# chjj/lcdb

Measured on AMD Instinct MI355X. Metric: device-resident GiB/s Snappy encode+decode, 4 KiB blocks, 1/2/4/8 MI355X, higher is better.
Workload: dtype u8

## Files before the change

lcdb_amd/csrc/lgs_api.cpp:

```cpp

#include <hip/hip_runtime.h>

#include <stdarg.h>
#include <stdint.h>
#include <stdio.h>
#include <stdlib.h>
#include <string.h>
#include <unistd.h>

#include <algorithm>
#include <atomic>
#include <chrono>
#include <condition_variable>
#include <deque>
#include <functional>
#include <memory>
#include <mutex>
#include <thread>
#include <unordered_map>
#include <vector>

#include "lgs_host.h"

namespace lgs {
// ... 1075 lines not shown
                        const uint32_t* d_key_len, const uint32_t* d_first, uint32_t nfilters,
                        int bits_per_key, uint8_t* d_out, const uint64_t* d_out_off,
                        void* stream) {
  if (nfilters == 0) return LGS_OK;
  if (!d_keys || !d_key_off || !d_key_len || !d_first || !d_out || !d_out_off)
    return fail(LGS_EINVAL, "NULL argument");
  if (bits_per_key < 0 || bits_per_key > kMaxBitsPerKey)
    return fail(LGS_EINVAL, "bits_per_key %d out of range", bits_per_key);
  LGS_HIP(launch_bloom_build(d_keys, d_key_off, d_key_len, d_first, nfilters,
                             (uint32_t)bits_per_key, bloom_k(bits_per_key), d_out, d_out_off,
                             0, (hipStream_t)stream));
  return LGS_OK;
}

int lgs_bloom_match_dev(const uint8_t* d_filters, const uint64_t* d_filter_off,
                        const uint32_t* d_filter_len, const uint32_t* d_query_filter,
                        const uint8_t* d_keys, const uint64_t* d_key_off,
                        const uint32_t* d_key_len, uint8_t* d_match, uint32_t nq, void* stream) {
  if (nq == 0) return LGS_OK;
  if (!d_filters || !d_filter_off || !d_filter_len || !d_query_filter || !d_keys || !d_key_off ||
      !d_key_len || !d_match)
    return fail(LGS_EINVAL, "NULL argument");
  LGS_HIP(launch_bloom_match(d_filters, d_filter_off, d_filter_len, d_query_filter, d_keys,
                             d_key_off, d_key_len, d_match, nq, (hipStream_t)stream));
  return LGS_OK;
}

int lgs_bloom_build_host(const uint8_t* keys, const uint64_t* key_off, const uint32_t* key_len,
                         const uint32_t* first, uint32_t nfilters, int bits_per_key,
                         uint8_t* out, const uint64_t* out_off) {
  if (nfilters == 0) return LGS_OK;
  if (!keys || !key_off || !key_len || !first || !out || !out_off)
    return fail(LGS_EINVAL, "NULL argument");
  if (bits_per_key < 0 || bits_per_key > kMaxBitsPerKey)
    return fail(LGS_EINVAL, "bits_per_key %d out of range", bits_per_key);
  for (uint32_t f = 0; f < nfilters; ++f)
    if (first[f + 1] < first[f]) return fail(LGS_EINVAL, "first[] decreases at filter %u", f);
  Lease lease(batch_pool());
  LGS_TRY(lease.acquire());
  Ctx& c = lease.ctx();
  const uint32_t nkeys = first[nfilters] - first[0];
  const uint32_t k0 = first[0];
  size_t key_bytes = 0, filt_bytes = 0;
  for (uint32_t i = k0; i < k0 + nkeys; ++i) key_bytes += key_len[i];
  for (uint32_t f = 0; f < nfilters; ++f)
    filt_bytes += lgs_bloom_filter_size(first[f + 1] - first[f], bits_per_key);
  Layout L;
  const size_t o_keys = L.take(key_bytes + 16);
  const size_t o_koff = L.take(8 * (size_t)nkeys);
  const size_t o_klen = L.take(4 * (size_t)nkeys);
  const size_t o_first = L.take(4 * ((size_t)nfilters + 1));
  const size_t o_foff = L.take(8 * (size_t)nfilters);
  const size_t up_end = L.at;
  const size_t o_filt = L.take(filt_bytes + 16);
  const size_t down_end = L.at;
  LGS_TRY(ctx_reserve(c, down_end, down_end));
  uint8_t* h = c.h_buf;
  uint8_t* d = c.d_buf;
  uint64_t* koff = (uint64_t*)(h + o_koff);
  uint32_t* klen = (uint32_t*)(h + o_klen);
  uint32_t* fst = (uint32_t*)(h + o_first);
  uint64_t* foff = (uint64_t*)(h + o_foff);
  size_t at = o_keys;
  for (uint32_t j = 0; j < nkeys; ++j) {
    memcpy(h + at, keys + key_off[k0 + j], key_len[k0 + j]);
    koff[j] = at;
    klen[j] = key_len[k0 + j];
    at += key_len[k0 + j];
  }
  memset(h + at, 0, 16);
  size_t fat = 0;
  for (uint32_t f = 0; f <= nfilters; ++f) fst[f] = first[f] - k0;
  for (uint32_t f = 0; f < nfilters; ++f) {
    foff[f] = fat;
    fat += lgs_bloom_filter_size(first[f + 1] - first[f], bits_per_key);
  }
  LGS_HIP(hipMemcpyAsync(d, h, up_end, hipMemcpyHostToDevice, c.stream));
  LGS_HIP(launch_bloom_build(d, (const uint64_t*)(d + o_koff), (const uint32_t*)(d + o_klen),
                             (const uint32_t*)(d + o_first), nfilters, (uint32_t)bits_per_key,
                             bloom_k(bits_per_key), d + o_filt, (const uint64_t*)(d + o_foff),
                             0, c.stream));
  LGS_HIP(hipMemcpyAsync(h + o_filt, d + o_filt, filt_bytes, hipMemcpyDeviceToHost, c.stream));
  LGS_HIP(hipStreamSynchronize(c.stream));
  for (uint32_t f = 0; f < nfilters; ++f)
    memcpy(out + out_off[f], h + o_filt + foff[f],
           lgs_bloom_filter_size(first[f + 1] - first[f], bits_per_key));
  return LGS_OK;
}

int lgs_bloom_match_host(const uint8_t* filters, const uint64_t* filter_off,
                         const uint32_t* filter_len, uint32_t nfilters,
                         const uint32_t* query_filter, const uint8_t* keys,
                         const uint64_t* key_off, const uint32_t* key_len, uint32_t nq,
                         uint8_t* match) {
  if (nq == 0) return LGS_OK;
  if (!filters || !filter_off || !filter_len || !query_filter || !keys || !key_off || !key_len ||
      !match)
    return fail(LGS_EINVAL, "NULL argument");
  for (uint32_t q = 0; q < nq; ++q)
    if (query_filter[q] >= nfilters)
      return fail(LGS_EINVAL, "query %u names filter %u of %u", q, query_filter[q], nfilters);
  Lease lease(batch_pool());
  LGS_TRY(lease.acquire());
  Ctx& c = lease.ctx();
  size_t fb = 0, kb = 0;
  for (uint32_t f = 0; f < nfilters; ++f) fb += filter_len[f];
  for (uint32_t q = 0; q < nq; ++q) kb += key_len[q];
  Layout L;
  const size_t o_f = L.take(fb + 16);
  const size_t o_foff = L.take(8 * (size_t)nfilters);
  const size_t o_flen = L.take(4 * (size_t)nfilters);
  const size_t o_qf = L.take(4 * (size_t)nq);
  const size_t o_k = L.take(kb + 16);
  const size_t o_koff = L.take(8 * (size_t)nq);
  const size_t o_klen = L.take(4 * (size_t)nq);
  const size_t up_end = L.at;
  const size_t o_m = L.take(nq);
  const size_t down_end = L.at;
  LGS_TRY(ctx_reserve(c, down_end, down_end));
  uint8_t* h = c.h_buf;
  uint8_t* d = c.d_buf;
  uint64_t* foff = (uint64_t*)(h + o_foff);
  uint32_t* flen = (uint32_t*)(h + o_flen);
  size_t at = 0;
  for (uint32_t f = 0; f < nfilters; ++f) {
    memcpy(h + o_f + at, filters + filter_off[f], filter_len[f]);
    foff[f] = at;
    flen[f] = filter_len[f];
    at += filter_len[f];
  }
  memset(h + o_f + at, 0, 16);
  memcpy(h + o_qf, query_filter, 4 * (size_t)nq);
  stage_keys(keys, key_off, key_len, nq, h + o_k, (uint64_t*)(h + o_koff), (uint32_t*)(h + o_klen));
  LGS_HIP(hipMemcpyAsync(d, h, up_end, hipMemcpyHostToDevice, c.stream));
  LGS_HIP(launch_bloom_match(d + o_f, (const uint64_t*)(d + o_foff), (const uint32_t*)(d + o_flen),
                             (const uint32_t*)(d + o_qf), d + o_k, (const uint64_t*)(d + o_koff),
                             (const uint32_t*)(d + o_klen), d + o_m, nq, c.stream));
  LGS_HIP(hipMemcpyAsync(h + o_m, d + o_m, nq, hipMemcpyDeviceToHost, c.stream));
  LGS_HIP(hipStreamSynchronize(c.stream));
  memcpy(match, h + o_m, nq);
  return LGS_OK;
}

int lgs_device_count(void) { return visible_devices(); }

int lgs_set_device(int device) {
  int count = lgs_device_count();
  if (device < 0 || device >= count)
    return fail(LGS_ENODEV, "device %d not present (%d visible)", device, count);
  t_want_device = device;
  return LGS_OK;
}

const char* lgs_last_error(void) { return t_err; }

const char* lgs_version(void) { return "lcdb_gpu_snappy 0.1 gfx950"; }

}
```

lcdb_amd/csrc/lgs_encode.hip:

```cpp
#include "lgs_device.h"
#include "lgs_probe_hooks.h"
#include "lgs_launch.h"
#include "lgs_service.h"

namespace lgs {

__constant__ ProbeTable kProbe = ProbeTable();

struct OutSlot {
  __amdgpu_buffer_rsrc_t r;
  __device__ void put(uint32_t soff, uint32_t voff, uint32_t v) const {
    __builtin_amdgcn_raw_buffer_store_b8((uint8_t)v, r, (int)voff, (int)soff, 0);
  }
  __device__ void put2(uint32_t soff, uint32_t voff, uint32_t v) const {
    __builtin_amdgcn_raw_buffer_store_b16((uint16_t)v, r, (int)voff, (int)soff, 0);
  }
  __device__ void put4(uint32_t soff, uint32_t voff, uint32_t v) const {
    __builtin_amdgcn_raw_buffer_store_b32(v, r, (int)voff, (int)soff, 0);
  }
  __device__ void put8(uint32_t soff, uint32_t voff, uint32_t lo, uint32_t hi) const {
    typedef uint32_t u32x2 __attribute__((ext_vector_type(2)));
    __builtin_amdgcn_raw_buffer_store_b64(u32x2{lo, hi}, r, (int)voff, (int)soff, 0);
  }
  __device__ void put16(uint32_t soff, uint32_t voff, u32x4 v) const {
    __builtin_amdgcn_raw_buffer_store_b128(v, r, (int)voff, (int)soff, 0);
  }
};

struct LdsIn {
  static constexpr bool kWin = false;
  const uint8_t* x;
  __device__ uint64_t rd64(uint32_t p) const { return lds_ld64(x, p); }
  __device__ Raw64 raw64(uint32_t p) const { return lds_raw64(x, p); }
  __device__ Raw32 raw32(uint32_t p) const { return lds_raw32(x, p); }
  __device__ uint32_t byte(uint32_t p) const { return x[p]; }
  __device__ u32x4 lit128(uint32_t p) const { return lds_ld128(x, p); }
  __device__ uint32_t litbyte(uint32_t p) const { return x[p]; }
  __device__ bool oow(uint32_t, uint32_t) const { return false; }
  __device__ void ensure(uint32_t) {}
  __device__ uint64_t g64(uint32_t) const { return 0; }
  __device__ uint32_t g32(uint32_t) const { return 0; }
  __device__ uint32_t gbyte(uint32_t) const { return 0; }
};

template <uint32_t W>
struct WinIn {
  static constexpr bool kWin = true;
  uint8_t* ring;
  gptr<const uint8_t> gal;
  uint32_t sh;
  uint32_t n;
  uint32_t hu;
  __device__ uint32_t ri(uint32_t p) const { return (p + sh) & (W - 1); }
  __device__ uint64_t rd64(uint32_t p) const { return lds_ld64(ring, ri(p)); }
  __device__ Raw64 raw64(uint32_t p) const { return lds_raw64(ring, ri(p)); }
  __device__ Raw32 raw32(uint32_t p) const { return lds_raw32(ring, ri(p)); }
  __device__ uint32_t byte(uint32_t p) const { return ring[ri(p)]; }
  __device__ bool oow(uint32_t p, uint32_t k) const {
    const uint32_t u = p + sh;
    return (u + W < hu) | (u + k > hu);
  }
  __device__ uint32_t gdw(uint32_t d) const {
    const uint32_t last = (n + sh - 1) >> 2;
    return *(gptr<const uint32_t>)(gal + 4 * (d < last ? d : last));
  }
  __device__ uint64_t g64(uint32_t p) const {
    const uint32_t u = p + sh, d = u >> 2, b = u & 3u;
    const uint32_t a = gdw(d), c = gdw(d + 1), e = gdw(d + 2);
    return ((uint64_t)__builtin_amdgcn_alignbyte(e, c, b) << 32) | __builtin_amdgcn_alignbyte(c, a, b);
  }
  __device__ uint32_t g32(uint32_t p) const {
    const uint32_t u = p + sh;
    return __builtin_amdgcn_alignbyte(gdw((u >> 2) + 1), gdw(u >> 2), u & 3u);
  }
  __device__ uint32_t gbyte(uint32_t p) const {
    const uint32_t u = p + sh;
    return (gdw(u >> 2) >> (8 * (u & 3u))) & 0xffu;
  }
  __device__ u32x4 lit128(uint32_t p) const {
    const uint32_t u = p + sh, d = u >> 2, b = u & 3u;
    const uint32_t a0 = gdw(d), a1 = gdw(d + 1), a2 = gdw(d + 2), a3 = gdw(d + 3), a4 = gdw(d + 4);
    return u32x4{__builtin_amdgcn_alignbyte(a1, a0, b), __builtin_amdgcn_alignbyte(a2, a1, b),
                 __builtin_amdgcn_alignbyte(a3, a2, b), __builtin_amdgcn_alignbyte(a4, a3, b)};
  }
  __device__ uint32_t litbyte(uint32_t p) const { return gbyte(p); }
  __device__ void stage() {
    const uint32_t lane = lane_id(), gend = (n + sh + 15) >> 4;
    u32x4 v[4];
#pragma unroll
    for (uint32_t j = 0; j < 4; ++j) {
      const uint32_t g = (hu >> 4) + lane + 64 * j;
      v[j] = g < gend ? *(gptr<const u32x4>)(gal + 16 * g) : u32x4{0, 0, 0, 0};
    }
    __builtin_amdgcn_s_waitcnt(0x0f70);
#pragma unroll
    for (uint32_t j = 0; j < 4; ++j) {
      const uint32_t r = (hu + 16 * (lane + 64 * j)) & (W - 1);
      *reinterpret_cast<u32x4*>(ring + r) = v[j];
      if (r < 16) *reinterpret_cast<u32x4*>(ring + W + r) = v[j];
    }
    order();
    hu += 4096;
  }
  __device__ void ensure(uint32_t P) {
    const uint32_t want = (P < n ? P : n) + sh;
    while (hu < want) stage();
  }
};

template <class IN>
__device__ __forceinline__ void copy_lit16(const OutSlot& o, uint32_t op, const IN& x,
                                           uint32_t to, uint32_t from, uint32_t len) {
  constexpr uint32_t kOff = 0x40000000u;
  const uint32_t lane = lane_id();
  const uint32_t whole = len & ~15u;
#pragma clang loop unroll(disable)
  for (uint32_t t0 = 0; t0 < whole; t0 += 4096) {
    u32x4 v[4];
#pragma unroll
    for (uint32_t k = 0; k < 4; ++k) {
      const uint32_t t = t0 + 1024 * k + 16 * lane;
      v[k] = x.lit128(from + (t < whole ? t : 0u));
    }
#pragma unroll
    for (uint32_t k = 0; k < 4; ++k) {
      const uint32_t t = t0 + 1024 * k + 16 * lane;
      o.put16(op, t < whole ? to + t : kOff, v[k]);
    }
  }
  const uint32_t rem = len - whole;
  if (rem) {
    u32x4 v = x.lit128(from + whole);
    uint32_t at = to + whole;
    const bool l0 = lane == 0;
    o.put8(op, l0 && (rem & 8) ? at : kOff, v.x, v.y);
    if (rem & 8) v = u32x4{v.z, v.w, 0, 0};
    at += rem & 8;
    o.put4(op, l0 && (rem & 4) ? at : kOff, v.x);
    if (rem & 4) v.x = v.y;
    at += rem & 4;
    o.put2(op, l0 && (rem & 2) ? at : kOff, v.x);
    if (rem & 2) v.x >>= 16;
    at += rem & 2;
    o.put(op, l0 && (rem & 1) ? at : kOff, v.x);
  }
}

template <class IN>
__device__ __forceinline__ uint32_t emit_literal(const OutSlot& o, uint32_t op, const IN& in,
                                                 uint32_t from, uint32_t len) {
  const uint32_t lane = lane_id();
  const uint32_t m = len - 1;
  const uint32_t hl = m < 60 ? 1u : (m < 256 ? 2u : 3u);
  const uint32_t h0 = m < 60 ? (m << 2) : (m < 256 ? 0xf0u : 0xf4u);
  const uint32_t hdr = h0 | ((m & 0xffu) << 8) | ((m >> 8) << 16);
  const uint32_t total = hl + len;
  if (IN::kWin || len > kWave) {
    if (lane < hl) o.put(op, lane, hdr >> (8 * lane));
    copy_lit16(o, op, in, hl, from, len);
    return total;
  }
#pragma clang loop unroll(disable) vectorize(disable)
  for (uint32_t j0 = 0; j0 < total; j0 += kWave) {
    const uint32_t j = j0 + lane;
    const uint32_t lb = in.litbyte(from + (j >= hl ? j - hl : 0));
    const uint32_t v = j < hl ? (hdr >> (8 * j)) : lb;
    if (j < total) o.put(op, j, v);
  }
  return total;
}

__device__ __forceinline__ uint32_t emit_copy(const OutSlot& o, uint32_t op, uint32_t dist,
                                              uint32_t len) {
  const uint32_t lane = lane_id();
  const uint8_t lo = (uint8_t)(dist & 0xffu), hi = (uint8_t)((dist >> 8) & 0xffu);
  if (len < 68) {
    const uint32_t has60 = len > 64 ? 1u : 0u;
    const uint32_t rest = len - 60 * has60;
    const bool c1 = rest < 12 && dist < 2048;
    const uint32_t first = c1 ? (((dist >> 8) << 5) | ((rest - 4) << 2) | 1u)
                              : (((rest - 1) << 2) | 2u);
    const uint32_t total = 3 * has60 + (c1 ? 2u : 3u);
    const uint32_t r = lane - 3 * has60;
    const uint32_t v = lane < 3 * has60 ? (lane == 0 ? 0xeeu : (lane == 1 ? lo : hi))
                                        : (r == 0 ? first : (r == 1 ? lo : hi));
    if (lane < total) o.put(op, lane, v);
    return total;
  }
  const uint32_t n64 = (len - 68) / 64 + 1;
  uint32_t rest = len - 64 * n64;
  const uint32_t has60 = rest > 64 ? 1u : 0u;
  rest -= 60 * has60;
  const bool c1 = rest < 12 && dist < 2048;
  const uint32_t head = 3 * (n64 + has60);
  const uint32_t total = head + (c1 ? 2u : 3u);
  const uint8_t last0 = c1 ? (uint8_t)(((dist >> 8) << 5) | ((rest - 4) << 2) | 1u)
                           : (uint8_t)(((rest - 1) << 2) | 2u);
#pragma clang loop unroll(disable) vectorize(disable)
  for (uint32_t b0 = 0; b0 < total; b0 += kWave) {
    const uint32_t b = b0 + lane;
    if (b < total) {
      uint8_t v;
      if (b < head) {
        const uint32_t r = b % 3;
        const bool is60 = has60 && b >= 3 * n64;
        v = r == 0 ? (is60 ? (uint8_t)0xee : (uint8_t)0xfe) : (r == 1 ? lo : hi);
      } else {
        const uint32_t r = b - head;
        v = r == 0 ? last0 : (r == 1 ? lo : hi);
      }
      o.put(op, b, v);
    }
  }
  return total;
}

constexpr uint32_t kLongLit = 256;

__device__ __forceinline__ void rec_lane(uint32_t& r, uint32_t v, uint64_t sel) {
  asm("v_cndmask_b32_e64 %0, %0, %1, %2" : "+v"(r) : "v"(v), "s"(sel));
}
template <class IN>
__device__ __forceinline__ uint32_t flush_ops(const OutSlot& o, uint32_t op, const IN& x,
                                              uint32_t recA, uint32_t recB, uint32_t k,
                                              uint32_t lit0) {
  const uint32_t lane = lane_id();
  const bool live = lane < k;
  const uint32_t base = recA & 0xffffu, clen = ((recA >> 16) - base) & 0xffffu, dist = base - recB;
  const uint32_t pend = (uint32_t)__shfl_up((int)(base + clen), 1);
  const uint32_t lit = lane == 0 ? lit0 : pend;
  const uint32_t LL = live ? base - lit : 0u;
  const uint32_t m = LL - 1;
  const uint32_t hl_big = m < 256 ? 2u : 3u;
  const uint32_t hl = LL == 0 ? 0u : (m < 60 ? 1u : hl_big);
  const uint32_t h0_big = m < 256 ? 0xf0u : 0xf4u;
  const uint32_t h0 = m < 60 ? (m << 2) : h0_big;
  const uint32_t hdr = h0 | ((m & 0xffu) << 8) | ((m >> 8) << 16);
  const bool longc = live && clen >= 68;
  const uint32_t has60 = clen > 64 ? 3u : 0u;
  const uint32_t rest = clen - 20 * has60;
  const bool c1 = rest < 12 && dist < 2048;
  const uint32_t first = c1 ? (((dist >> 8) << 5) | ((rest - 4) << 2) | 1u)
                            : (((rest - 1) << 2) | 2u);
  uint32_t ntag = has60 + (c1 ? 2u : 3u);
  if (longc) {
    const uint32_t n64 = (clen - 68) / 64 + 1;
    uint32_t r = clen - 64 * n64;
    const uint32_t h60 = r > 64 ? 1u : 0u;
    r -= 60 * h60;
    ntag = 3 * (n64 + h60) + ((r < 12 && dist < 2048) ? 2u : 3u);
  }
  const uint32_t size = live ? hl + LL + ntag : 0u;
  uint32_t incl = size;
#pragma unroll
  for (uint32_t d = 1; d < kWave; d <<= 1) {
    const uint32_t t = (uint32_t)__shfl_up((int)incl, d);
    incl += lane >= d ? t : 0u;
  }
  const uint32_t excl = incl - size;
  const uint32_t total = lane_val(incl, kWave - 1);
  const uint32_t lat = excl + hl;
  const uint32_t tat = lat + LL;
  constexpr uint32_t kOff = 0x40000000u;
  const uint32_t LLs = LL > kLongLit ? 0u : LL;
  const uint32_t whole = LLs & ~15u;
#pragma clang loop unroll(disable)
  for (uint32_t t = 0; ballot(t < whole); t += 16) {
    const bool on = t < whole;
    o.put16(op, on ? lat + t : kOff, x.lit128(on ? lit + t : 0u));
  }
  {
    const uint32_t rem = LLs - whole;
    u32x4 v = x.lit128(LLs ? lit + whole : 0u);
    uint32_t at = lat + whole;
    o.put8(op, (rem & 8) ? at : kOff, v.x, v.y);
    if (rem & 8) v = u32x4{v.z, v.w, 0, 0};
    at += rem & 8;
    o.put4(op, (rem & 4) ? at : kOff, v.x);
    if (rem & 4) v.x = v.y;
    at += rem & 4;
    o.put2(op, (rem & 2) ? at : kOff, v.x);
    if (rem & 2) v.x >>= 16;
    at += rem & 2;
    o.put(op, (rem & 1) ? at : kOff, v.x);
  }
  for (uint64_t big = ballot(LL > kLongLit); big; big &= big - 1) {
    const uint32_t l = (uint32_t)__builtin_ctzll(big);
    const uint32_t from = lane_val(lit, l), len = lane_val(LL, l), to = lane_val(lat, l);
    copy_lit16(o, op, x, to, from, len);
  }
  o.put(op, hl > 0 ? excl : kOff, hdr);
  o.put(op, hl > 1 ? excl + 1 : kOff, hdr >> 8);
  o.put(op, hl > 2 ? excl + 2 : kOff, hdr >> 16);
  const bool shortc = live && !longc;
  const uint32_t fb = tat + has60;
  o.put(op, shortc && has60 ? tat : kOff, 0xeeu);
  o.put(op, shortc && has60 ? tat + 1 : kOff, dist);
  o.put(op, shortc && has60 ? tat + 2 : kOff, dist >> 8);
  o.put(op, shortc ? fb : kOff, first);
  o.put(op, shortc ? fb + 1 : kOff, dist);
  o.put(op, shortc && !c1 ? fb + 2 : kOff, dist >> 8);
  for (uint64_t lc = ballot(longc); lc; lc &= lc - 1) {
    const uint32_t l = (uint32_t)__builtin_ctzll(lc);
    emit_copy(o, op + lane_val(tat, l), lane_val(dist, l), lane_val(clen, l));
  }
  return op + total;
}

__host__ __device__ constexpr uint32_t probe_off(uint32_t k) {
  return k + (k > 32 ? k - 32 : 0u) + (k > 48 ? k - 48 : 0u) + (k > 59 ? k - 59 : 0u);
}
constexpr uint32_t kProbeClosed = 67;
constexpr bool probe_off_matches_table() {
  constexpr ProbeTable t;
  for (uint32_t k = 0; k <= kProbeClosed; ++k)
    if (probe_off(k) != t.off[k]) return false;
  return true;
}
static_assert(probe_off_matches_table(), "closed-form probe schedule != snappy.c:138-143");

constexpr uint32_t kSink = kTableCap;

__device__ __forceinline__ uint32_t lds_addr(const void* p) {
  return (uint32_t)(uintptr_t)(const __attribute__((address_space(3))) uint8_t*)p;
}

template <uint32_t TAB>
__device__ __forceinline__ uint32_t lds_mskor_rtn(uint32_t a, uint32_t mask, uint32_t data) {
  uint32_t old;
  asm volatile("ds_mskor_rtn_b32 %0, %1, %2, %3 offset:%4\n\ts_waitcnt lgkmcnt(0)"
               : "=v"(old) : "v"(a), "v"(mask), "v"(data), "i"(TAB) : "memory");
  return old;
}
template <uint32_t TAB>
__device__ __forceinline__ void lds_mskor(uint32_t a, uint32_t mask, uint32_t data) {
  asm volatile("ds_mskor_b32 %0, %1, %2 offset:%3" : : "v"(a), "v"(mask), "v"(data), "i"(TAB)
               : "memory");
}

struct PostLanes {
  uint32_t e0, e1, bm;
};
constexpr uint32_t kProbesPerBatch = kWave - 2;
__device__ __forceinline__ PostLanes post_lanes(uint32_t lane) {
  const uint32_t pk = lane >= 2 ? lane - 2 : 0;
  return PostLanes{lane == 0 ? 0xfffffffeu : (lane == 1 ? 0xffffffffu : probe_off(pk)),
                   lane < 2 ? 0u : probe_off(pk + 1), lane == 1 ? 0xffffffu : 0u};
}
constexpr uint32_t kPostLast = probe_off(kProbesPerBatch - 1);

template <uint32_t TAB, class IN>
__device__ __forceinline__ uint32_t encode_chunk(IN& x, uint32_t n, uint16_t* tab,
                                                 const OutSlot& o, uint32_t op0,
                                                 const PostLanes& pl) {
  const uint32_t lane = lane_id();
  const uint32_t last = n - kMargin;

  uint32_t tsize = 256, shift = 24;
  while (tsize < kTableCap && tsize < n) {
    tsize <<= 1;
    --shift;
  }
  for (uint32_t e = lane; e < tsize / 8; e += kWave)
    reinterpret_cast<u32x4*>(tab)[e] = u32x4{0, 0, 0, 0};
  order();
  const uint32_t hsh = shift - 1;
  constexpr uint32_t kSinkOff = 2 * kSink;

  uint32_t op = op0;
  uint32_t at = 0;
  uint32_t start = 1;
  uint32_t kb = 0;
  uint32_t recA = 0, recB = 0, lit0 = 0;
  uint64_t sel = 1;

  uint32_t p;
  uint64_t vmask = 0;
  Raw64 xr;
  uint32_t prev = 0, h2 = 0, ta = 0, sh = 0, mask = 0;
  auto batch = [&](bool valid) -> uint64_t {
    vmask = ballot(valid);
    uint32_t xv = xr.lo(), xh = xr.hi();
    if constexpr (IN::kWin) {
      const bool o8 = valid & x.oow(p, 8);
      if (ballot(o8)) {
        const uint64_t g = x.g64(p);
        xv = o8 ? (uint32_t)g : xv;
        xh = o8 ? (uint32_t)(g >> 32) : xh;
      }
    }
    h2 = (xv * kHashMul) >> hsh;
    ta = valid ? (h2 & ~3u) : kSinkOff;
    sh = (h2 << 3) & 16u;
    mask = 0xffffu << sh;
    const uint32_t old = lds_mskor_rtn<TAB>(ta, mask, p << sh);
    prev = (old >> sh) & 0xffffu;
    Raw32 yr = x.raw32(prev);
    if (LGS_ENC_REPLAY(prev > p, vmask)) {
      const uint32_t p0 = lane_val(p, (uint32_t)__builtin_ctzll(vmask));
      lds_mskor<TAB>(prev < p0 ? ta : kSinkOff, mask, prev << sh);
      for (uint64_t r = vmask; r; r &= r - 1) {
        const uint32_t l = (uint32_t)__builtin_ctzll(r);
        const uint32_t got = lds_mskor_rtn<TAB>(lane == l ? ta : kSinkOff, mask, p << sh);
        prev = lane == l ? (got >> sh) & 0xffffu : prev;
      }
      yr = x.raw32(prev);
    }
    uint32_t yv = yr.value();
    if constexpr (IN::kWin) {
      const bool o4 = valid & x.oow(prev, 4);
      if (ballot(o4)) yv = o4 ? x.g32(prev) : yv;
    }
    return ballot(((xv ^ yv) | (xh & pl.bm)) == 0) & vmask & ~1ull;
  };
  bool evalid = (lane >= 2) & (pl.e1 <= last - 1);
  p = evalid ? 1 + pl.e0 : 0;
  if constexpr (IN::kWin) x.ensure(1 + kPostLast + 16);
  xr = x.raw64(p);
  for (;;) {
    const uint32_t at_in = at;
    for (uint64_t mm = batch(evalid); mm;
         mm = batch((int32_t)(last - start) >= (int32_t)pl.e1)) {
      const uint32_t m = (uint32_t)__builtin_ctzll(mm);
      const uint32_t base = lane_val(p, m);
      const uint32_t ref = lane_val(prev, m);
      *reinterpret_cast<uint16_t*>(reinterpret_cast<uint8_t*>(tab) +
                                   (((lane > m) & (prev <= base)) ? (ta | (h2 & 2u)) : kSinkOff)) =
          (uint16_t)prev;
      const uint32_t dist = base - ref;
      uint32_t at_n = base + 4;
#pragma clang loop unroll(disable)
      for (;;) {
        const uint32_t q = at_n + lane;
        if constexpr (IN::kWin) x.ensure(at_n + kWave);
        uint32_t bq = x.byte(q), br = x.byte(q - dist);
        if constexpr (IN::kWin) {
          const bool orq = x.oow(q - dist, 1) || x.oow(q, 1);
          if (ballot(orq)) {
            br = orq ? x.gbyte(q - dist) : br;
            bq = orq ? x.gbyte(q) : bq;
          }
        }
        const uint64_t diff = ballot(br != bq) | ballot(q >= n);
        if (diff) {
          at_n += (uint32_t)__builtin_ctzll(diff);
          break;
        }
        at_n += kWave;
      }
      start = at_n + 1;
      p = start + pl.e0;
      if constexpr (IN::kWin) x.ensure(start + kPostLast + 16);
      xr = x.raw64(p);
      at = at_n;
      rec_lane(recA, base | (at_n << 16), sel);
      rec_lane(recB, ref, sel);
      sel <<= 1;
      if (!sel) {
        op = flush_ops(o, op, x, recA, recB, kWave, lit0);
        sel = 1;
        lit0 = at_n;
      }
    }
    if (at >= last) break;
    if ((vmask | 3ull) != ~0ull) break;
    kb = (at != at_in ? 0u : kb) + kProbesPerBatch;
    const uint32_t kk = kb + lane - 2;
    const bool in_tab = (lane >= 2) & (kk < kProbeTab);
    const uint32_t kc = in_tab ? kk : 0u;
    const uint32_t o0 = kProbe.off[kc], o1 = kProbe.off[kc + 1];
    __builtin_amdgcn_s_waitcnt(0x0f70);
    evalid = in_tab & (o1 <= last - start);
    p = evalid ? start + o0 : 0;
    if constexpr (IN::kWin) x.ensure(start + lane_val(o0, kWave - 1) + 16);
    xr = x.raw64(p);
  }
  const uint32_t nops = (uint32_t)__builtin_ctzll(sel);
  if (nops) op = flush_ops(o, op, x, recA, recB, nops, lit0);

  if (at < n) op += emit_literal(o, op, x, at, n - at);
  return op;
}

__device__ __forceinline__ uint32_t emit_header(const OutSlot& o, uint32_t hv) {
  if (hv == 0xffffffffu) return 0;
  const uint32_t lane = lane_id();
  const uint32_t hl = hv < (1u << 7) ? 1 : hv < (1u << 14) ? 2 : hv < (1u << 21) ? 3
                    : hv < (1u << 28) ? 4 : 5;
  if (lane < hl) {
    uint32_t b = (hv >> (7 * lane)) & 0x7fu;
    if (lane + 1 < hl) b |= 0x80u;
    o.put(0, lane, b);
  }
  return hl;
}

__device__ __forceinline__ OutSlot out_slot(uint8_t* out, uint64_t off, uint32_t len) {
  return OutSlot{__builtin_amdgcn_make_buffer_rsrc(out + off, 0, (int)(32 + len + len / 6),
                                                   0x00020000)};
}

template <uint32_t IMG>
struct EncLds {
  static_assert(IMG % 16 == 0 && IMG <= 65535 - 2 * kSink - 16, "table offset");
  uint8_t img[IMG];
  uint16_t tab[kTableCap + 8];
};

template <uint32_t IN_CAP>
__device__ __forceinline__ uint32_t encode_item(EncLds<IN_CAP + 112>& s, gptr<const uint8_t> src,
                                                uint32_t len, uint32_t hv, const OutSlot& o) {
  constexpr uint32_t kImg = IN_CAP + 112;
  const PostLanes pl = post_lanes(lane_id());
  LGS_ENC_PH_DECL;
  uint32_t op = emit_header(o, hv);

  for (uint32_t c0 = 0; c0 < len; c0 += kChunk) {
    const uint32_t clen = len - c0 < kChunk ? len - c0 : kChunk;
    constexpr uint32_t kR = (IN_CAP + 16 + 1023) / 1024 < 8 ? (IN_CAP + 16 + 1023) / 1024 : 8;
    stage_in_linear<kR>(s.img, src + c0, clen);
    LdsIn x{s.img};
    order();
    LGS_ENC_PH_STAGED();
    if (clen >= kMinBlock) {
      op = encode_chunk<kImg>(x, clen, s.tab, o, op, pl);
    } else {
      op += emit_literal(o, op, x, 0, clen);
    }
    order();
  }
  LGS_ENC_PH_END(o, len);
  return op;
}

#ifndef LGS_ENCODE_SERVICE_ONLY
template <uint32_t IN_CAP>
__global__ __launch_bounds__(64) void encode_kernel(
    const uint8_t* __restrict__ in, const uint64_t* __restrict__ in_off,
    const uint32_t* __restrict__ in_len, uint8_t* __restrict__ out,
    const uint64_t* __restrict__ out_off, uint32_t* __restrict__ out_len,
    const uint32_t* __restrict__ hdr, const uint32_t* __restrict__ index, uint32_t n,
    const uint32_t* __restrict__ count, const Item1 one) {
  __shared__ __attribute__((aligned(16))) EncLds<IN_CAP + 112> s;
  if (lds_addr(&s) != 0) __builtin_trap();

  const uint32_t slot = blockIdx.x;
  if (slot >= (count ? uni(*count) : n)) return;
  const uint32_t i = uni(index ? index[slot] : slot);

  uint64_t ioff, ooff;
  uint32_t len, hv;
  if (one.on) {
    ioff = one.in_off; ooff = one.out_off; len = one.in_len; hv = one.aux;
  } else {
    ioff = uni64(in_off[i]); ooff = uni64(out_off[i]); len = uni(in_len[i]);
    hv = uni(hdr ? hdr[i] : len);
  }
  const uint32_t op = encode_item<IN_CAP>(s, to_global(in) + ioff, len, hv, out_slot(out, ooff, len));
  if (lane_id() == 0) out_len[i] = op;
}

#endif

#ifndef LGS_ENCODE_BATCH_ONLY
__global__ __launch_bounds__(64) void encode_service_kernel(SvcMailbox* __restrict__ mb,
                                                            uint64_t idle,
                                                            SvcControl* __restrict__ ctl) {
  __shared__ __attribute__((aligned(16))) EncLds<kSvcMaxItem + 112> s;
  if (lds_addr(&s) != 0) __builtin_trap();
  svc_loop(mb + blockIdx.x, idle, ctl,
           [&](uint32_t len, uint64_t input, uint64_t arena, uint32_t* status, uint32_t* out_len) {
             uint8_t* a = reinterpret_cast<uint8_t*>(arena);
             len = len < kSvcMaxItem ? len : kSvcMaxItem;
             *out_len = encode_item<kSvcMaxItem>(s, to_global(reinterpret_cast<const uint8_t*>(input)),
                                                 len, len, out_slot(a, kSvcOut, len));
             *status = 1;
           });
}

hipError_t launch_encode_service(SvcMailbox* mb, uint32_t nslots, uint64_t idle,
                                 SvcControl* ctl, hipStream_t s) {
  hipLaunchKernelGGL(encode_service_kernel, dim3(nslots), dim3(64), 0, s, mb, idle, ctl);
  return hipGetLastError();
}
#endif

#ifndef LGS_ENCODE_SERVICE_ONLY
template <uint32_t W>
__global__ __launch_bounds__(64) void encode_win_kernel(
    const uint8_t* __restrict__ in, const uint64_t* __restrict__ in_off,
    const uint32_t* __restrict__ in_len, uint8_t* __restrict__ out,
    const uint64_t* __restrict__ out_off, uint32_t* __restrict__ out_len,
    const uint32_t* __restrict__ hdr, const uint32_t* __restrict__ index, uint32_t n,
    const uint32_t* __restrict__ count) {
  __shared__ __attribute__((aligned(16))) EncLds<W + 16> s;
  if (lds_addr(&s) != 0) __builtin_trap();

  const uint32_t slot = blockIdx.x;
  if (slot >= (count ? uni(*count) : n)) return;
  const uint32_t i = uni(index ? index[slot] : slot);
  const uint32_t lane = lane_id();
  const PostLanes pl = post_lanes(lane);
  const uint32_t len = uni(in_len[i]);
  const gptr<const uint8_t> src = to_global(in) + uni64(in_off[i]);
  const OutSlot o = out_slot(out, uni64(out_off[i]), len);
  uint32_t op = emit_header(o, uni(hdr ? hdr[i] : len));
  for (uint32_t c0 = 0; c0 < len; c0 += kChunk) {
    const uint32_t clen = len - c0 < kChunk ? len - c0 : kChunk;
    const gptr<const uint8_t> g = src + c0;
    const uint32_t sh = (uint32_t)(reinterpret_cast<uintptr_t>(g) & 15u);
    WinIn<W> x{s.img, g - sh, sh, clen, 0};
    if (clen >= kMinBlock) {
      x.ensure(W / 4);
      op = encode_chunk<W + 16>(x, clen, s.tab, o, op, pl);
    } else {
      op += emit_literal(o, op, x, 0, clen);
    }
    __builtin_amdgcn_s_waitcnt(0x0f70);
    order();
  }
  if (lane == 0) out_len[i] = op;
}

static hipError_t launch_encode_big(const EncodeArgs& a, hipStream_t s);

template <uint32_t IN_CAP>
static hipError_t launch_encode_cls(const EncodeArgs& a, hipStream_t s) {
  hipLaunchKernelGGL((encode_kernel<IN_CAP>), dim3(a.n), dim3(64), 0, s, a.in,
                     a.in_off, a.in_len, a.out, a.out_off, a.out_len, a.hdr, a.index, a.n,
                     a.count, a.one);
  return hipGetLastError();
}

constexpr uint32_t kEncCap0 = 4608;
// ... 43 lines not shown
```

lcdb_amd/csrc/lgs_launch.h:

```cpp
#pragma once

#include <hip/hip_runtime.h>
#include <stddef.h>
#include <stdint.h>

#include <atomic>

namespace lgs {

enum DecodeKernel {
  kDecAuto = 0, kDecRing = 1, kDecWave = 2, kDecQuad = 3, kDecOps = 4, kDecGroup = 5, kDecChain = 6,
  kDecRing32 = 7
};
enum WideKernel { kWideWalk = 0, kWideTrips = 1, kWideGroup = 2 };
struct Options {
  std::atomic<int> decoder{kDecAuto};
  std::atomic<int> split{1};
  std::atomic<int> wide{0};
  std::atomic<int> verify_overlap{1};
};
Options& options();

struct Item1 {
  uint64_t in_off = 0, out_off = 0;
  uint32_t in_len = 0, aux = 0;
  uint32_t on = 0;
};

struct DecodeArgs {
  const uint8_t* in; const uint64_t* in_off; const uint32_t* in_len;
  uint8_t* out; const uint64_t* out_off; const uint32_t* out_cap;
  uint32_t* out_len; uint8_t* status; const uint32_t* index; uint32_t n;
  const uint32_t* count;
  Item1 one{};
};

struct EncodeArgs {
  const uint8_t* in; const uint64_t* in_off; const uint32_t* in_len;
  uint8_t* out; const uint64_t* out_off; uint32_t* out_len;
  const uint32_t* hdr; const uint32_t* index; uint32_t n;
  const uint32_t* count;
  Item1 one{};
};

hipError_t launch_decode(const DecodeArgs& a, uint32_t max_out, hipStream_t s);
#ifdef LGS_PROBE_DECODERS
hipError_t launch_decode_quad(const DecodeArgs& a, hipStream_t s);
hipError_t launch_decode_ops(const DecodeArgs& a, hipStream_t s);
hipError_t launch_decode_trips(const DecodeArgs& a, hipStream_t s);
hipError_t launch_decode_ring32(const DecodeArgs& a, hipStream_t s);
#endif
hipError_t launch_decode_pair(const DecodeArgs& a, hipStream_t s);

#ifdef LGS_PROBE_DECODERS
constexpr uint32_t kGroupMaxOut = 66048;
hipError_t launch_decode_group(const DecodeArgs& a, uint32_t max_out, hipStream_t s);
constexpr uint32_t kChainMaxOut = 16896;
hipError_t launch_decode_chain(const DecodeArgs& a, uint32_t max_out, hipStream_t s);
#endif
hipError_t launch_encode(const EncodeArgs& a, uint32_t max_in, hipStream_t s);
constexpr uint32_t kSplitMinBlocks = 512;
hipError_t launch_classify(const uint32_t* len, uint32_t n, uint32_t b0, uint32_t b1, uint32_t b2,
                           uint32_t* list, uint32_t* cnt, hipStream_t s);
class Scratch {
 public:
  Scratch(size_t bytes, hipStream_t s);
  ~Scratch() { (void)release(); }
  Scratch(const Scratch&) = delete;
  Scratch& operator=(const Scratch&) = delete;
  hipError_t status() const { return err_; }
  void* get() const { return p_; }
  hipError_t release() {
    void* p = p_;
    p_ = nullptr;
    return p ? hipFreeAsync(p, s_) : hipSuccess;
  }

 private:
  void* p_ = nullptr;
  hipStream_t s_;
  hipError_t err_;
};

constexpr uint32_t kSvcMaxSlots = 64;
constexpr uint32_t kSvcMaxItem = 4608;
constexpr uint32_t kSvcIn = 0;
constexpr uint32_t kSvcOut = 8192;

struct alignas(128) SvcMailbox {
  uint32_t req;
  uint32_t len;
  uint32_t aux;
  uint32_t stop;
  uint64_t arena;
  uint64_t pad0[5];
  uint32_t ack;
  uint32_t status;
  uint32_t out_len;
  uint32_t pad1[13];
};
static_assert(sizeof(SvcMailbox) == 128, "mailbox layout");

struct alignas(64) SvcControl {
  uint64_t activity;
  uint64_t closing;
  uint64_t pad[6];
};

hipError_t launch_encode_service(SvcMailbox* mb, uint32_t nslots, uint64_t idle,
                                 SvcControl* ctl, hipStream_t s);
hipError_t launch_decode_service(SvcMailbox* mb, uint32_t nslots, uint64_t idle,
                                 SvcControl* ctl, hipStream_t s);


constexpr uint32_t kStCorrupt = 0, kStOk = 1, kStNoSpace = 2, kStIoErr = 3, kStBadCrc = 4,
                   kStBadType = 5;

struct FrameArgs {
  const uint8_t* raw; const uint64_t* raw_off; const uint32_t* raw_len;
  const uint8_t* enc; const uint64_t* enc_off; const uint32_t* enc_len;
  uint8_t* file; uint64_t base; const uint64_t* foff;
  uint64_t* handle_off; uint64_t* handle_size; uint32_t n;
};

struct CheckArgs {
  const uint8_t* file; uint64_t file_len; const uint64_t* hoff; const uint64_t* hsize;
  uint32_t verify; uint8_t* out; const uint64_t* out_off; const uint32_t* out_cap;
  uint32_t* out_len; uint8_t* status;
  uint64_t* dec_in_off; uint32_t* dec_len; uint64_t* dec_off; uint32_t* dec_cap;
  uint64_t dummy_off; uint32_t n;
};

hipError_t launch_crc(const uint8_t* in, const uint64_t* in_off, const uint32_t* in_len,
                      const uint8_t* type, int masked, uint32_t* crc, uint32_t n, hipStream_t s);
size_t scan_parts(uint32_t n);
hipError_t launch_scan(int mode, const uint32_t* raw_len, const uint32_t* enc_len, uint64_t* part,
                       uint64_t base, uint64_t* off, uint64_t* end, uint32_t n, hipStream_t s);
hipError_t launch_frame(const FrameArgs& a, hipStream_t s);
hipError_t launch_pack(const uint8_t* src, const uint64_t* src_off, const uint32_t* len,
                       uint8_t* dst, const uint64_t* dst_off, uint32_t n, hipStream_t s);
hipError_t launch_check(const CheckArgs& a, hipStream_t s);
hipError_t launch_merge(uint8_t* status, uint32_t* out_len, const uint8_t* dec_status,
                        const uint32_t* dec_out_len, const uint8_t* bad, uint32_t n,
                        hipStream_t s);
hipError_t launch_verify(const uint8_t* file, uint64_t file_len, const uint64_t* hoff,
                         const uint64_t* hsize, uint8_t* bad, uint32_t n, hipStream_t s);


hipError_t launch_bloom_build(const uint8_t* keys, const uint64_t* key_off,
                              const uint32_t* key_len, const uint32_t* first, uint32_t nfilters,
                              uint32_t bpk, uint32_t k, uint8_t* out, const uint64_t* out_off,
                              uint32_t trim, hipStream_t s);
hipError_t launch_bloom_match(const uint8_t* filters, const uint64_t* filter_off,
                              const uint32_t* filter_len, const uint32_t* qfilter,
                              const uint8_t* keys, const uint64_t* key_off,
                              const uint32_t* key_len, uint8_t* match, uint32_t nq,
                              hipStream_t s);
hipError_t launch_filter_block_build(const uint8_t* keys, const uint64_t* key_off,
                                     const uint32_t* key_len, const uint32_t* block_first,
                                     const uint64_t* block_off, uint32_t nblocks,
                                     uint64_t data_end, uint32_t bpk, uint32_t k, uint32_t trim,
                                     uint8_t* out, uint64_t* size, uint32_t* kf, uint64_t* foff,
                                     uint64_t* part, uint32_t* meta, hipStream_t s);
size_t filter_block_parts(uint64_t data_end);
hipError_t launch_filter_block_match(const uint8_t* blk, uint64_t n, const uint64_t* qoff,
                                     const uint8_t* keys, const uint64_t* key_off,
                                     const uint32_t* key_len, uint32_t trim, uint8_t* match,
                                     uint32_t nq, hipStream_t s);

hipError_t launch_hbm_copy(void* dst, const void* src, size_t bytes, hipStream_t s);

int set_error(int code, const char* msg);

}
```

lcdb_amd/csrc/lgs_probe_hooks.h:

```cpp
#pragma once

#include <stdint.h>

#ifdef LGS_PROBE_RING_PHASES
#define LGS_RING_PH_DECL                                   \
  uint32_t ph_[8] = {0, 0, 0, 0, 0, 0, 0, 0};               \
  uint32_t ph_trips_ = 0;                                   \
  uint64_t ph_t_ = __builtin_amdgcn_s_memtime()
#define LGS_RING_PH(k)                                     \
  do {                                                     \
    const uint64_t t_ = __builtin_amdgcn_s_memtime();      \
    ph_[k] += (uint32_t)(t_ - ph_t_);                      \
    ph_t_ = t_;                                            \
  } while (0)
#define LGS_RING_PH_TRIP() (++ph_trips_)
__device__ __forceinline__ uint32_t lgs_ring_ph_value_(const uint32_t* ph, uint32_t trips,
                                                       uint32_t lane, uint32_t dflt) {
  uint32_t v = lane == 8 ? trips : dflt;
#pragma unroll
  for (uint32_t k = 0; k < 8; ++k) v = lane == k ? ph[k] : v;
  return v;
}
#else
#define LGS_RING_PH_DECL do {} while (0)
#define LGS_RING_PH(k) do {} while (0)
#define LGS_RING_PH_TRIP() do {} while (0)
#endif

#ifdef LGS_PROBE_RING_PHASES
#define LGS_PAIR_PH_DECL LGS_RING_PH_DECL
#define LGS_PAIR_PH(k) LGS_RING_PH(k)
#define LGS_PAIR_PH_TRIP() LGS_RING_PH_TRIP()
#define LGS_PAIR_PH_END_MOVER(ok, lane, ptr)                              \
  do {                                                                    \
    if ((ok) && (lane) <= 8) *(ptr) = lgs_ring_ph_value_(ph_, ph_trips_, (lane), 0u); \
    __builtin_amdgcn_s_waitcnt(0x0f70);                                   \
    pair_barrier();                                                       \
  } while (0)
#define LGS_PAIR_PH_END_WALKER(ok, lane, ptr)                             \
  do {                                                                    \
    pair_barrier();                                                       \
    if ((ok) && (lane) >= 16 && (lane) <= 24)                             \
      *(ptr) = lgs_ring_ph_value_(ph_, ph_trips_, (lane) - 16, 0u);       \
  } while (0)
#else
#define LGS_PAIR_PH_DECL do {} while (0)
#define LGS_PAIR_PH(k) do {} while (0)
#define LGS_PAIR_PH_TRIP() do {} while (0)
#define LGS_PAIR_PH_END_MOVER(ok, lane, ptr) do {} while (0)
#define LGS_PAIR_PH_END_WALKER(ok, lane, ptr) do {} while (0)
#endif

#ifdef LGS_PROBE_NOFAR
#define LGS_RING_FAR_LD16(p) ((void)(p), u32x4{0, 0, 0, 0})
#else
#define LGS_RING_FAR_LD16(p) ld16(p)
#endif
#ifdef LGS_PROBE_NOFLUSH
#define LGS_RING_FLUSH_ST(g, v, c) \
  do { if ((v).x == 0x12345678u && (c) == 77777u) st16((g), (v)); } while (0)
#else
#define LGS_RING_FLUSH_ST(g, v, c) \
  do { if ((c) >= 16) st16((g), (v)); else st_exact((g), (v), (c)); } while (0)
#endif

#ifdef LGS_PROBE_DEC_TIMING
#define LGS_DEC_PH_DECL                                                   \
  const uint64_t dtp0_ = __builtin_amdgcn_s_memtime();                    \
  const uint64_t drt0_ = __builtin_amdgcn_s_memrealtime();                \
  uint64_t dtp1_ = dtp0_
#define LGS_DEC_PH_STAGED()                                               \
  do { __builtin_amdgcn_s_waitcnt(0); dtp1_ = __builtin_amdgcn_s_memtime(); } while (0)
#define LGS_DEC_PH_END(FLUSH_STMT, STORE_PTR)                             \
  do {                                                                    \
    __builtin_amdgcn_s_waitcnt(0);                                        \
    const uint64_t tp2_ = __builtin_amdgcn_s_memtime();                   \
    FLUSH_STMT;                                                           \
    __builtin_amdgcn_s_waitcnt(0);                                        \
    const uint64_t tp3_ = __builtin_amdgcn_s_memtime();                   \
    const uint64_t rt3_ = __builtin_amdgcn_s_memrealtime();               \
    if (lane_id() == 0) {                                                 \
      gptr<uint32_t> q_ = (STORE_PTR);                                    \
      q_[0] = (uint32_t)(dtp1_ - dtp0_);                                  \
      q_[1] = (uint32_t)(tp2_ - dtp1_);                                   \
      q_[2] = (uint32_t)(tp3_ - tp2_);                                    \
      q_[3] = (uint32_t)(rt3_ - drt0_);                                   \
    }                                                                     \
  } while (0)
#else
#define LGS_DEC_PH_DECL do {} while (0)
#define LGS_DEC_PH_STAGED() do {} while (0)
#define LGS_DEC_PH_END(FLUSH_STMT, STORE_PTR) do {} while (0)
#endif

#ifdef LGS_PROBE_FORCE_REPLAY
#define LGS_ENC_REPLAY(cond, vmask) (vmask)
#else
#define LGS_ENC_REPLAY(cond, vmask) (ballot(cond) & (vmask))
#endif
#ifdef LGS_PROBE_ENC_TIMING
#define LGS_ENC_PH_DECL                                                   \
  const uint64_t etp0_ = __builtin_amdgcn_s_memtime();                    \
  uint64_t etp1_ = etp0_
#define LGS_ENC_PH_STAGED()                                               \
  do { __builtin_amdgcn_s_waitcnt(0); etp1_ = __builtin_amdgcn_s_memtime(); } while (0)
#define LGS_ENC_PH_END(SLOT, LEN)                                         \
  do {                                                                    \
    __builtin_amdgcn_s_waitcnt(0);                                        \
    const uint64_t tp2_ = __builtin_amdgcn_s_memtime();                   \
    if (lane_id() == 0) {                                                 \
      const uint32_t b_ = 32 + (LEN) + (LEN) / 6 - 16;                    \
      (SLOT).put4(0, b_, (uint32_t)(etp1_ - etp0_));                      \
      (SLOT).put4(0, b_ + 4, (uint32_t)(tp2_ - etp1_));                   \
      (SLOT).put4(0, b_ + 8, 0x7e57u);                                    \
    }                                                                     \
  } while (0)
#else
#define LGS_ENC_PH_DECL do {} while (0)
#define LGS_ENC_PH_STAGED() do {} while (0)
#define LGS_ENC_PH_END(SLOT, LEN) do {} while (0)
#endif
```

Measured before the change: 326.9.

## Replace per-batch hash replay with optimistic pass and serial fallback re-encode

The encoder no longer runs a per-batch serialized replay when a hash-table slot returns a position ahead of the current one. It runs an optimistic parallel pass, records whether any such conflict happened, and if so restarts the window and re-encodes the whole chunk with a serial table-update variant. It also biases positions by a constant so distance and end arithmetic fold into fewer ops, and records ops with v_writelane instead of a shifting select mask. The branch is removed from the common path, but any chunk that hits a conflict is now encoded twice.

```diff
diff --git a/lcdb_amd/csrc/lgs_api.cpp b/lcdb_amd/csrc/lgs_api.cpp
--- a/lcdb_amd/csrc/lgs_api.cpp
+++ b/lcdb_amd/csrc/lgs_api.cpp
@@ -1251,6 +1251,14 @@
   return LGS_OK;
 }
 
+#ifdef LGS_PROBE_DECODERS
+int lgs_probe_encode_second_pass(int on) {
+  LGS_HIP(enc_second_pass_batch(on != 0));
+  LGS_HIP(enc_second_pass_service(on != 0));
+  return LGS_OK;
+}
+#endif
+
 const char* lgs_last_error(void) { return t_err; }
 
 const char* lgs_version(void) { return "lcdb_gpu_snappy 0.1 gfx950"; }
diff --git a/lcdb_amd/csrc/lgs_encode.hip b/lcdb_amd/csrc/lgs_encode.hip
--- a/lcdb_amd/csrc/lgs_encode.hip
+++ b/lcdb_amd/csrc/lgs_encode.hip
@@ -6,6 +6,17 @@
 namespace lgs {
 
 __constant__ ProbeTable kProbe = ProbeTable();
+
+#ifdef LGS_PROBE_DECODERS
+static __device__ uint32_t lgs_enc_second_pass = 0;
+#ifdef LGS_ENCODE_SERVICE_ONLY
+hipError_t enc_second_pass_service(uint32_t on) {
+#else
+hipError_t enc_second_pass_batch(uint32_t on) {
+#endif
+  return hipMemcpyToSymbol(HIP_SYMBOL(lgs_enc_second_pass), &on, sizeof(on));
+}
+#endif
 
 struct OutSlot {
   __amdgpu_buffer_rsrc_t r;
@@ -38,6 +49,7 @@
   __device__ uint32_t litbyte(uint32_t p) const { return x[p]; }
   __device__ bool oow(uint32_t, uint32_t) const { return false; }
   __device__ void ensure(uint32_t) {}
+  __device__ void restart() {}
   __device__ uint64_t g64(uint32_t) const { return 0; }
   __device__ uint32_t g32(uint32_t) const { return 0; }
   __device__ uint32_t gbyte(uint32_t) const { return 0; }
@@ -105,6 +117,10 @@
   __device__ void ensure(uint32_t P) {
     const uint32_t want = (P < n ? P : n) + sh;
     while (hu < want) stage();
+  }
+  __device__ void restart() {
+    hu = 0;
+    ensure(W / 4);
   }
 };
 
@@ -216,9 +232,12 @@
 }
 
 constexpr uint32_t kLongLit = 256;
-
-__device__ __forceinline__ void rec_lane(uint32_t& r, uint32_t v, uint64_t sel) {
-  asm("v_cndmask_b32_e64 %0, %0, %1, %2" : "+v"(r) : "v"(v), "s"(sel));
+constexpr uint32_t kEndBias = kWave - 4;
+
+__device__ __forceinline__ void rec_lane(uint32_t& a, uint32_t& b, uint32_t va, uint32_t vb,
+                                         uint32_t k) {
+  asm("s_mov_b32 m0, %4\n\tv_writelane_b32 %0, %2, m0\n\tv_writelane_b32 %1, %3, m0"
+      : "+v"(a), "+v"(b) : "s"(va), "s"(vb), "s"(k) : "m0");
 }
 template <class IN>
 __device__ __forceinline__ uint32_t flush_ops(const OutSlot& o, uint32_t op, const IN& x,
@@ -226,7 +245,8 @@
                                               uint32_t lit0) {
   const uint32_t lane = lane_id();
   const bool live = lane < k;
-  const uint32_t base = recA & 0xffffu, clen = ((recA >> 16) - base) & 0xffffu, dist = base - recB;
+  const uint32_t base = recA & 0xffffu, clen = ((recA >> 16) - kEndBias - base) & 0xffffu,
+                 dist = 0u - recB;
   const uint32_t pend = (uint32_t)__shfl_up((int)(base + clen), 1);
   const uint32_t lit = lane == 0 ? lit0 : pend;
   const uint32_t LL = live ? base - lit : 0u;
@@ -339,20 +359,22 @@
 }
 
 struct PostLanes {
-  uint32_t e0, e1, bm;
+  uint32_t e0, e1, bm, vu, l4;
 };
 constexpr uint32_t kProbesPerBatch = kWave - 2;
 __device__ __forceinline__ PostLanes post_lanes(uint32_t lane) {
   const uint32_t pk = lane >= 2 ? lane - 2 : 0;
-  return PostLanes{lane == 0 ? 0xfffffffeu : (lane == 1 ? 0xffffffffu : probe_off(pk)),
-                   lane < 2 ? 0u : probe_off(pk + 1), lane == 1 ? 0xffffffu : 0u};
+  constexpr uint32_t s0 = 1u - kEndBias;
+  return PostLanes{lane == 0 ? s0 - 2 : (lane == 1 ? s0 - 1 : s0 + probe_off(pk)),
+                   lane < 2 ? s0 : s0 + probe_off(pk + 1), lane == 1 ? 0xffffffu : 0u,
+                   lane == 0 ? 0u : 0xffffffffu, lane + 4};
 }
 constexpr uint32_t kPostLast = probe_off(kProbesPerBatch - 1);
 
-template <uint32_t TAB, class IN>
-__device__ __forceinline__ uint32_t encode_chunk(IN& x, uint32_t n, uint16_t* tab,
-                                                 const OutSlot& o, uint32_t op0,
-                                                 const PostLanes& pl) {
+template <uint32_t TAB, class IN, bool SERIAL>
+__device__ __forceinline__ uint32_t encode_pass(IN& x, uint32_t n, uint16_t* tab,
+                                                const OutSlot& o, uint32_t op0,
+                                                const PostLanes& pl, bool& broke) {
   const uint32_t lane = lane_id();
   const uint32_t last = n - kMargin;
 
@@ -368,16 +390,16 @@
   constexpr uint32_t kSinkOff = 2 * kSink;
 
   uint32_t op = op0;
-  uint32_t at = 0;
-  uint32_t start = 1;
+  uint32_t am = kEndBias;
   uint32_t kb = 0;
   uint32_t recA = 0, recB = 0, lit0 = 0;
-  uint64_t sel = 1;
+  uint32_t kop = 0;
+  uint64_t bad = 0;
 
   uint32_t p;
   uint64_t vmask = 0;
   Raw64 xr;
-  uint32_t prev = 0, h2 = 0, ta = 0, sh = 0, mask = 0;
+  uint32_t prev = 0, h2 = 0, ta = 0;
   auto batch = [&](bool valid) -> uint64_t {
     vmask = ballot(valid);
     uint32_t xv = xr.lo(), xh = xr.hi();
@@ -391,80 +413,76 @@
     }
     h2 = (xv * kHashMul) >> hsh;
     ta = valid ? (h2 & ~3u) : kSinkOff;
-    sh = (h2 << 3) & 16u;
-    mask = 0xffffu << sh;
-    const uint32_t old = lds_mskor_rtn<TAB>(ta, mask, p << sh);
-    prev = (old >> sh) & 0xffffu;
-    Raw32 yr = x.raw32(prev);
-    if (LGS_ENC_REPLAY(prev > p, vmask)) {
-      const uint32_t p0 = lane_val(p, (uint32_t)__builtin_ctzll(vmask));
-      lds_mskor<TAB>(prev < p0 ? ta : kSinkOff, mask, prev << sh);
+    const uint32_t sh = (h2 << 3) & 16u;
+    const uint32_t mask = 0xffffu << sh;
+    if constexpr (SERIAL) {
+      prev = 0;
       for (uint64_t r = vmask; r; r &= r - 1) {
         const uint32_t l = (uint32_t)__builtin_ctzll(r);
         const uint32_t got = lds_mskor_rtn<TAB>(lane == l ? ta : kSinkOff, mask, p << sh);
         prev = lane == l ? (got >> sh) & 0xffffu : prev;
       }
-      yr = x.raw32(prev);
-    }
+    } else {
+      const uint32_t old = lds_mskor_rtn<TAB>(ta, mask, p << sh);
+      prev = vec((old >> sh) & 0xffffu);
+    }
+    const Raw32 yr = x.raw32(prev);
+    if constexpr (!SERIAL) bad |= ballot(prev > p) & vmask;
+    const uint32_t w = vec((xh & pl.bm) | ~(valid ? pl.vu : 0u));
     uint32_t yv = yr.value();
     if constexpr (IN::kWin) {
       const bool o4 = valid & x.oow(prev, 4);
       if (ballot(o4)) yv = o4 ? x.g32(prev) : yv;
     }
-    return ballot(((xv ^ yv) | (xh & pl.bm)) == 0) & vmask & ~1ull;
+    return ballot(((xv ^ yv) | w) == 0);
   };
-  bool evalid = (lane >= 2) & (pl.e1 <= last - 1);
-  p = evalid ? 1 + pl.e0 : 0;
+  const uint32_t lim = last - (pl.e1 - pl.e0);
+  bool evalid = (lane >= 2) & ((int32_t)(last - am) >= (int32_t)pl.e1);
+  p = evalid ? am + pl.e0 : 0;
   if constexpr (IN::kWin) x.ensure(1 + kPostLast + 16);
   xr = x.raw64(p);
   for (;;) {
-    const uint32_t at_in = at;
+    const uint32_t am_in = am;
     for (uint64_t mm = batch(evalid); mm;
-         mm = batch((int32_t)(last - start) >= (int32_t)pl.e1)) {
+         mm = batch((int32_t)p <= (int32_t)lim)) {
       const uint32_t m = (uint32_t)__builtin_ctzll(mm);
       const uint32_t base = lane_val(p, m);
-      const uint32_t ref = lane_val(prev, m);
+      const uint32_t ndm = lane_val(prev, m) - base;
       *reinterpret_cast<uint16_t*>(reinterpret_cast<uint8_t*>(tab) +
                                    (((lane > m) & (prev <= base)) ? (ta | (h2 & 2u)) : kSinkOff)) =
           (uint16_t)prev;
-      const uint32_t dist = base - ref;
-      uint32_t at_n = base + 4;
+      uint32_t a = base;
+      uint64_t diff;
 #pragma clang loop unroll(disable)
-      for (;;) {
-        const uint32_t q = at_n + lane;
-        if constexpr (IN::kWin) x.ensure(at_n + kWave);
-        uint32_t bq = x.byte(q), br = x.byte(q - dist);
+      do {
+        const uint32_t q = vec(a + pl.l4);
+        if constexpr (IN::kWin) x.ensure(a + 4 + kWave);
+        uint32_t bq = x.byte(q), br = x.byte(q + ndm);
         if constexpr (IN::kWin) {
-          const bool orq = x.oow(q - dist, 1) || x.oow(q, 1);
+          const bool orq = x.oow(q + ndm, 1) || x.oow(q, 1);
           if (ballot(orq)) {
-            br = orq ? x.gbyte(q - dist) : br;
+            br = orq ? x.gbyte(q + ndm) : br;
             bq = orq ? x.gbyte(q) : bq;
           }
         }
-        const uint64_t diff = ballot(br != bq) | ballot(q >= n);
-        if (diff) {
-          at_n += (uint32_t)__builtin_ctzll(diff);
-          break;
-        }
-        at_n += kWave;
+        diff = ballot(br != bq) | ballot(q >= n);
+        a += kWave;
+      } while (!diff);
+      am = a + (uint32_t)__builtin_ctzll(diff);
+      p = am + pl.e0;
+      if constexpr (IN::kWin) x.ensure(am - kEndBias + 1 + kPostLast + 16);
+      xr = x.raw64(p);
+      rec_lane(recA, recB, base | (am << 16), ndm, kop);
+      if (++kop == kWave) {
+        op = flush_ops(o, op, x, recA, recB, kWave, lit0);
+        kop = 0;
+        lit0 = am - kEndBias;
       }
-      start = at_n + 1;
-      p = start + pl.e0;
-      if constexpr (IN::kWin) x.ensure(start + kPostLast + 16);
-      xr = x.raw64(p);
-      at = at_n;
-      rec_lane(recA, base | (at_n << 16), sel);
-      rec_lane(recB, ref, sel);
-      sel <<= 1;
-      if (!sel) {
-        op = flush_ops(o, op, x, recA, recB, kWave, lit0);
-        sel = 1;
-        lit0 = at_n;
-      }
-    }
-    if (at >= last) break;
+    }
+    if (am - kEndBias >= last) break;
     if ((vmask | 3ull) != ~0ull) break;
-    kb = (at != at_in ? 0u : kb) + kProbesPerBatch;
+    kb = (am != am_in ? 0u : kb) + kProbesPerBatch;
+    const uint32_t start = am - kEndBias + 1;
     const uint32_t kk = kb + lane - 2;
     const bool in_tab = (lane >= 2) & (kk < kProbeTab);
     const uint32_t kc = in_tab ? kk : 0u;
@@ -475,11 +493,25 @@
     if constexpr (IN::kWin) x.ensure(start + lane_val(o0, kWave - 1) + 16);
     xr = x.raw64(p);
   }
-  const uint32_t nops = (uint32_t)__builtin_ctzll(sel);
-  if (nops) op = flush_ops(o, op, x, recA, recB, nops, lit0);
-
+  if (kop) op = flush_ops(o, op, x, recA, recB, kop, lit0);
+
+  broke = bad != 0;
+  const uint32_t at = am - kEndBias;
   if (at < n) op += emit_literal(o, op, x, at, n - at);
   return op;
+}
+
+template <uint32_t TAB, class IN>
+__device__ __forceinline__ uint32_t encode_chunk(IN& x, uint32_t n, uint16_t* tab,
+                                                 const OutSlot& o, uint32_t op0,
+                                                 const PostLanes& pl) {
+  bool broke;
+  const uint32_t op = encode_pass<TAB, IN, false>(x, n, tab, o, op0, pl, broke);
+  if (!LGS_ENC_REPLAY(broke)) return op;
+  __builtin_amdgcn_s_waitcnt(0x0f70);
+  order();
+  x.restart();
+  return encode_pass<TAB, IN, true>(x, n, tab, o, op0, pl, broke);
 }
 
 __device__ __forceinline__ uint32_t emit_header(const OutSlot& o, uint32_t hv) {
diff --git a/lcdb_amd/csrc/lgs_launch.h b/lcdb_amd/csrc/lgs_launch.h
--- a/lcdb_amd/csrc/lgs_launch.h
+++ b/lcdb_amd/csrc/lgs_launch.h
@@ -59,6 +59,10 @@
 hipError_t launch_decode_chain(const DecodeArgs& a, uint32_t max_out, hipStream_t s);
 #endif
 hipError_t launch_encode(const EncodeArgs& a, uint32_t max_in, hipStream_t s);
+#ifdef LGS_PROBE_DECODERS
+hipError_t enc_second_pass_batch(uint32_t on);
+hipError_t enc_second_pass_service(uint32_t on);
+#endif
 constexpr uint32_t kSplitMinBlocks = 512;
 hipError_t launch_classify(const uint32_t* len, uint32_t n, uint32_t b0, uint32_t b1, uint32_t b2,
                            uint32_t* list, uint32_t* cnt, hipStream_t s);
diff --git a/lcdb_amd/csrc/lgs_probe_hooks.h b/lcdb_amd/csrc/lgs_probe_hooks.h
--- a/lcdb_amd/csrc/lgs_probe_hooks.h
+++ b/lcdb_amd/csrc/lgs_probe_hooks.h
@@ -93,10 +93,12 @@
 #define LGS_DEC_PH_END(FLUSH_STMT, STORE_PTR) do {} while (0)
 #endif
 
-#ifdef LGS_PROBE_FORCE_REPLAY
-#define LGS_ENC_REPLAY(cond, vmask) (vmask)
+#if defined(LGS_PROBE_FORCE_REPLAY)
+#define LGS_ENC_REPLAY(broke) ((void)(broke), true)
+#elif defined(LGS_PROBE_DECODERS)
+#define LGS_ENC_REPLAY(broke) ((broke) | (__builtin_amdgcn_readfirstlane(lgs_enc_second_pass) != 0))
 #else
-#define LGS_ENC_REPLAY(cond, vmask) (ballot(cond) & (vmask))
+#define LGS_ENC_REPLAY(broke) (broke)
 #endif
 #ifdef LGS_PROBE_ENC_TIMING
 #define LGS_ENC_PH_DECL                                                   \
```

Result: faster. 333.9, median of 6 (+2.1%).
